# rapidsai/cugraph-gnn

Measured on AMD Instinct MI355X. Metric: sampled-edges/sec (sample+renumber+feature-gather+SAGEConv fwd), ogbn-products-like fan-out [25, 10], higher is better.
Workload: dtype int64 ids (int32 timed as a variant) + f32 features (SAGE lin_l/lin_r product: bf16x3-split MFMA, f32 accumulate); 1 GPU; ogbn-products-like RMAT: V=2449029, E=118462496 directed (CSR row_ptr i64 / col i64 replicated per GPU), feat fp32 [V,100], batch 1024/GPU, fan-out [25, 10], 2-layer SAGEConv(mean) 100-256-47 fwd, step = 8 call groups of 188 mini-batches; parallelism=dp1 (seeds sharded, no data-path collective)

## Files before the change

cugraph-gnn_amd/csrc/wg_sage_mfma.hip:

```cpp
#include "wg_sage_mfma_parts.hpp"

namespace wgamd {
namespace {
using namespace sage_mfma;

template <int TR>
__device__ __forceinline__ void consume_tile(const mfma_args& a, int64_t tile, const float* tile_lds, int cw, int lane,
                                             float* scratch)
{
  constexpr int RT = TR / 32;
  f32x16 c[RT][2];
#pragma unroll
  for (int rt = 0; rt < RT; rt++)
#pragma unroll
    for (int ct = 0; ct < 2; ct++)
#pragma unroll
      for (int i = 0; i < 16; i++) c[rt][ct][i] = 0.f;
  const int lm = lane & 31, lh = lane >> 5;
  const float* a_lane      = tile_lds + lm * a.SD + lh * 8;
  const float* b_lane = a.w_tiles + ((int64_t)(cw * 64 + lm)) * 16 + lh * 8;
  braw_t b0, b1;
  bfrag_t fb;
  araw_t<RT> raw;
  afrag_t<RT> fa;
  load_b(b0, b_lane, a.N, 0);
  for (int ks = 0; ks < a.KS; ks += 2) {
    load_a_raw<RT>(raw, a_lane, a.SD, ks);
    if (ks + 1 < a.KS) load_b(b1, b_lane, a.N, ks + 1);
    split_a<RT>(raw, fa);
    split_b(b0, fb);
    mma_frags<RT>(c, fa, fb);
    if (ks + 1 < a.KS) {
      load_a_raw<RT>(raw, a_lane, a.SD, ks + 1);
      if (ks + 2 < a.KS) load_b(b0, b_lane, a.N, ks + 2);
      split_a<RT>(raw, fa);
      split_b(b1, fb);
      mma_frags<RT>(c, fa, fb);
    }
  }
  epilogue<RT>(a, c, tile * TR, cw, lane, scratch);
}

template <int HEAD, int BODY, int VALU_PER>
__device__ __forceinline__ void mfma_valu_interleave()
{
#pragma unroll
  for (int i = 0; i < HEAD; i++) __builtin_amdgcn_sched_group_barrier(0x008, 1, 0);
#pragma unroll
  for (int i = 0; i < BODY; i++) {
    __builtin_amdgcn_sched_group_barrier(0x008, 1, 0);
    __builtin_amdgcn_sched_group_barrier(0x002, VALU_PER, 0);
  }
}

template <int RT, int AD, typename LoadA>
__device__ __forceinline__ void consume_range(const mfma_args& a, f32x16 (&c)[RT][2], bfrag_t (&b)[3], int ks0, int ks1, int cw,
                                              int lane, LoadA load_a)
{
  const int lm = lane & 31, lh = lane >> 5;
  const int64_t b_plane_dw = (int64_t)a.KS * a.N * 8;
  const uint32_t* b_lane   = reinterpret_cast<const uint32_t*>(a.w_tiles) + ((int64_t)(cw * 64 + lm)) * 8 + lh * 4;
  araw_t<RT> raw[AD];
  afrag_t<RT> fa[2];
  const int kl = ks1 - 1;
  load_a(raw[0], ks0);
  if constexpr (AD == 2) load_a(raw[1], ks0 + 1 < kl ? ks0 + 1 : kl);
  split_a<RT>(raw[0], fa[0]);
  auto step = [&](auto I, int ks) {
    constexpr int i = decltype(I)::value;
    load_a(raw[i % AD], ks + AD < kl ? ks + AD : kl);
    int kb = ks + 2;
    kb     = kb >= a.KS ? kb - a.KS : kb;
    load_b_planes(b[(i + 2) % 3], b_lane, b_plane_dw, a.N, kb);
    mma_frags<RT>(c, fa[i & 1], b[i % 3]);
    split_a<RT>(raw[(i + 1) % AD], fa[(i + 1) & 1]);
    mfma_valu_interleave<4, 6 * RT * 2 - 4, 5>();
    __builtin_amdgcn_sched_barrier(0);
  };
  int ks = ks0;
  for (; ks + 5 < ks1; ks += 6) {
    step(std::integral_constant<int, 0>{}, ks);
    step(std::integral_constant<int, 1>{}, ks + 1);
    step(std::integral_constant<int, 2>{}, ks + 2);
    step(std::integral_constant<int, 3>{}, ks + 3);
    step(std::integral_constant<int, 4>{}, ks + 4);
    step(std::integral_constant<int, 5>{}, ks + 5);
  }
  const int r = ks1 - ks;
  if (r > 0) step(std::integral_constant<int, 0>{}, ks);
  if (r > 1) step(std::integral_constant<int, 1>{}, ks + 1);
  if (r > 2) step(std::integral_constant<int, 2>{}, ks + 2);
  if (r > 3) step(std::integral_constant<int, 3>{}, ks + 3);
  if (r > 4) step(std::integral_constant<int, 4>{}, ks + 4);
  const int rot = (ks1 - ks0) % 3;
  if (rot == 1) {
    const bfrag_t t = b[0];
    b[0] = b[1], b[1] = b[2], b[2] = t;
  } else if (rot == 2) {
    const bfrag_t t = b[0];
    b[0] = b[2], b[2] = b[1], b[1] = t;
  }
}

constexpr int kPD = 2;
__host__ __device__ constexpr int b_slot(int ks) { return ks < kPD ? ks : kPD + (ks % kPD); }
__host__ __device__ constexpr int w_lds_ksteps(int FC)
{
#ifdef WG_NO_WLDS
  return 0;
#endif
  const int tiles = (2 * 64 * row_stride_dw(FC) + 16 + 4 * kScratchDw + 16) * 4;
  const int free_ = 160 * 1024 - tiles;
  const int ks    = free_ / (256 * 64);
  return ks < 0 ? 0 : (ks > 4 ? 4 : ks);
}

template <int TR, int FC>
struct static_consumer {
  static constexpr int RT = TR / 32, KSC = (2 * FC + 15) / 16, SD = row_stride_dw(FC);
  static constexpr int KL = TR == 64 ? w_lds_ksteps(FC) : 0;
  braw_t bb[2 * kPD];
  uint32_t b_lane_off;
  const float* w_lds;
  f32x16 c[RT][2];

  __device__ __forceinline__ void load_b_static(const mfma_args& a, braw_t& f, int ks) const
  {
#ifdef WG_ABL_NO_B
    return;
#endif
#ifdef WG_ABL_HALF_B
    if (ks & 1) return;
#endif
    if (ks >= KSC - KL) {
#pragma unroll
      for (int ct = 0; ct < 2; ct++)
#pragma unroll
        for (int h = 0; h < 2; h++)
          f.v[ct][h] = *reinterpret_cast<const f32x4*>(w_lds + (((ks - (KSC - KL)) * 2 + ct) * 2 + h) * 256);
      return;
    }
    const char* wb = reinterpret_cast<const char*>(a.w_tiles);
#pragma unroll
    for (int ct = 0; ct < 2; ct++) {
      const size_t at = ((size_t)ks * a.N + ct * 32) * 64 + b_lane_off;
      f.v[ct][0]      = *reinterpret_cast<const f32x4*>(wb + at);
      f.v[ct][1]      = *reinterpret_cast<const f32x4*>(wb + at + 16);
    }
  }

  __device__ __forceinline__ void prime(const mfma_args& a, int cw, int lane, float* w_lds_wave)
  {
    b_lane_off = (uint32_t)(((cw * 64 + (lane & 31)) * 16 + (lane >> 5) * 8) * 4);
    w_lds      = w_lds_wave + lane * 4;
    if constexpr (KL > 0) {
      const char* wb = reinterpret_cast<const char*>(a.w_tiles);
#pragma unroll
      for (int ks = KSC - KL; ks < KSC; ks++)
#pragma unroll
        for (int ct = 0; ct < 2; ct++)
#pragma unroll
          for (int h = 0; h < 2; h++)
            *reinterpret_cast<f32x4*>(const_cast<float*>(w_lds) + (((ks - (KSC - KL)) * 2 + ct) * 2 + h) * 256) =
              *reinterpret_cast<const f32x4*>(wb + ((size_t)ks * a.N + ct * 32) * 64 + b_lane_off + h * 16);
    }
#pragma unroll
    for (int j = 0; j < kPD; j++) load_b_static(a, bb[j], j);
  }

  __device__ __forceinline__ void multiply(const mfma_args& a, const float* tile_lds, int lane)
  {
#pragma unroll
    for (int rt = 0; rt < RT; rt++)
#pragma unroll
      for (int ct = 0; ct < 2; ct++)
#pragma unroll
        for (int i = 0; i < 16; i++) c[rt][ct][i] = 0.f;
    const float* a_lane = tile_lds + (lane & 31) * SD + (lane >> 5) * 8;
    araw_t<RT> raw;
    afrag_t<RT> fa[2];
    load_a_raw<RT>(raw, a_lane, SD, 0);
    split_a<RT>(raw, fa[0]);
#pragma unroll
    for (int ks = 0; ks < KSC; ks++) {
      if (ks + 1 < KSC) load_a_raw<RT>(raw, a_lane, SD, ks + 1);
      bfrag_t fb;
      split_b(bb[b_slot(ks)], fb);
      mma_frags<RT>(c, fa[ks & 1], fb);
      const int nk = ks + kPD;
      if (nk < KSC) load_b_static(a, bb[b_slot(nk)], nk);
      else load_b_static(a, bb[nk - KSC], nk - KSC);
      if (ks + 1 < KSC) split_a<RT>(raw, fa[(ks + 1) & 1]);
      __builtin_amdgcn_sched_barrier(0);
    }
  }
  __device__ __forceinline__ void store(const mfma_args& a, int64_t tile, int cw, int lane, float* scratch)
  {
    epilogue<RT>(a, c, tile * TR, cw, lane, scratch);
  }
};

template <typename IdT, int LG, int TR, int CW, bool OFF32, int FC, bool HALF = false>
__global__ void __launch_bounds__((CW + kProducerWaves) * 64)
sage_layer_mfma_kernel(mfma_args a)
{
  static_assert(!HALF || FC == 0, "the half-tile mode runs the runtime-shape consumer");
  extern __shared__ __attribute__((aligned(16))) float lds[];
  const int tile_dw = TR * a.SD;
  for (int i = threadIdx.x; i < 2 * tile_dw + 16; i += blockDim.x) lds[i] = 0.f;
  __syncthreads();
  const int lane = threadIdx.x & 63;
  int wave = threadIdx.x >> 6;
  if (a.debug & 64) {
    uint32_t* keys = reinterpret_cast<uint32_t*>(lds + 2 * tile_dw + 16 + CW * kScratchDw);
    const int simd = (int)__builtin_amdgcn_s_getreg((1 << 11) | (4 << 6) | 4);
    if (lane == 0) keys[wave] = (uint32_t)(((simd & 1) * 2 + (simd >> 1)) * 16 + wave);
    __syncthreads();
    const uint32_t mine_key = keys[wave];
    int rank = 0;
#pragma unroll
    for (int w = 0; w < CW + kProducerWaves; w++) rank += keys[w] < mine_key ? 1 : 0;
    wave = __builtin_amdgcn_readfirstlane(rank);
    __syncthreads();
  }
  const int64_t n_tiles = (a.n_rows + TR - 1) / TR;
  const int64_t mine    = blockIdx.x < n_tiles ? (n_tiles - blockIdx.x + gridDim.x - 1) / gridDim.x : 0;
  auto tile_of          = [&](int64_t n) { return (int64_t)blockIdx.x + n * gridDim.x; };
  auto stamp            = [&](int64_t n, int which) {
    if (a.stamps && blockIdx.x == 0 && lane == 0 && n < 64) a.stamps[(n * 8 + wave) * 2 + which] = __builtin_readcyclecounter();
  };

  if constexpr (HALF) {
    const int KSh = a.KS / 2;
    if (wave >= CW) {
      using P     = producer<IdT, LG, 32, OFF32, true>;
      using off_t = typename P::off_t;
      constexpr int IT = P::IT, kNb = P::kNb, kDepth = P::kDepth;
      static_assert(TR == 64, "two 32-row sub-tiles per tile");
      P p(a, wave - CW, lane);
      bounds_t<IT> b_next;
      ids_t<IT> i_next;
      meta_t<IT, off_t> cur;
      f32x4 buf[kDepth][kNb + 1];
      auto sub_of = [&](int64_t j) { return 2 * tile_of(j >> 1) + (j & 1); };
      p.load_bounds(sub_of(0), b_next);
      p.load_ids(sub_of(0), b_next, i_next);
      p.finish(i_next, cur);
#pragma unroll
      for (int it = 0; it < kDepth - 1; it++) p.issue(cur, it, buf[it]);
      constexpr int kHalf = IT / 2;
      for (int64_t n = 0; n <= mine; n++) {
        if (n < mine && !(a.debug & 2)) {
          float* tile_lds = lds + (n & 1) * tile_dw;
#pragma unroll
          for (int sub = 0; sub < 2; sub++) {
            const int64_t j = 2 * n + sub;
            float* rows_lds = tile_lds + sub * 32 * a.SD;
            p.load_bounds(sub_of(j + 1), b_next);
#pragma unroll
            for (int it = 0; it < IT; it++) {
              if (it == kHalf) p.load_ids(sub_of(j + 1), b_next, i_next);
              if (it + kDepth - 1 < IT) p.issue(cur, it + kDepth - 1, buf[(it + kDepth - 1) % kDepth]);
              p.reduce_store(cur, it, buf[it % kDepth], rows_lds);
            }
            p.second_window(cur, rows_lds);
            p.long_rows(sub_of(j), cur, rows_lds);
            p.finish(i_next, cur);
            if (j + 1 < 2 * mine) {
#pragma unroll
              for (int it = 0; it < kDepth - 1; it++) p.issue(cur, it, buf[it]);
            }
          }
        }
        lds_barrier();
      }
    } else {
      constexpr int RT = TR / 32;
      float* scratch = lds + 2 * tile_dw + 16 + wave * kScratchDw;
      f32x16 c[RT][2];
      bfrag_t b[3];
      {
        const uint32_t* b_lane =
          reinterpret_cast<const uint32_t*>(a.w_tiles) + ((int64_t)(wave * 64 + (lane & 31))) * 8 + (lane >> 5) * 4;
        load_b_planes(b[0], b_lane, (int64_t)a.KS * a.N * 8, a.N, 0);
        load_b_planes(b[1], b_lane, (int64_t)a.KS * a.N * 8, a.N, 1);
      }
      const IdT* src_ids = static_cast<const IdT*>(a.src_ids);
      for (int64_t n = 0; n <= mine; n++) {
        if (n >= 1 && !(a.debug & 1)) {
          const int64_t row0 = tile_of(n - 1) * TR;
          const float* self_ptr[RT];
#pragma unroll
          for (int rt = 0; rt < RT; rt++) {
            const int64_t row  = row0 + rt * 32 + (lane & 31);
            const int64_t srow = a.self_rows[row < a.n_rows ? row : a.n_rows - 1];
            self_ptr[rt]       = reinterpret_cast<const float*>(reinterpret_cast<const char*>(a.x) + table_row<IdT>(src_ids, srow) * a.row_scale) +
                           (lane >> 5) * 8;
          }
#pragma unroll
          for (int rt = 0; rt < RT; rt++)
#pragma unroll
            for (int ct = 0; ct < 2; ct++)
#pragma unroll
              for (int i = 0; i < 16; i++) c[rt][ct][i] = 0.f;
          store_agg<TR, CW>(a, lds + ((n - 1) & 1) * tile_dw, row0, wave, lane);
          const float* a_lane = lds + ((n - 1) & 1) * tile_dw + (lane & 31) * a.SD + (lane >> 5) * 8;
          consume_range<RT, 1>(a, c, b, 0, KSh, wave, lane, [&](araw_t<RT>& f, int ks) { load_a_raw<RT>(f, a_lane, a.SD, ks); });
          consume_range<RT, 2>(a, c, b, KSh, a.KS, wave, lane, [&](araw_t<RT>& f, int ks) {
#pragma unroll
            for (int rt = 0; rt < RT; rt++) {
              const float* p = self_ptr[rt] + (ks - KSh) * 16;
              f.v[rt][0]     = *reinterpret_cast<const f32x4*>(p);
              f.v[rt][1]     = *reinterpret_cast<const f32x4*>(p + 4);
            }
          });
          epilogue<RT>(a, c, row0, wave, lane, scratch);
        }
        lds_barrier();
      }
    }
  } else if (wave >= CW) {
    if (a.debug & 16) __builtin_amdgcn_s_setprio(3);
    using P     = producer<IdT, LG, TR, OFF32>;
    using off_t = typename P::off_t;
    constexpr int IT = P::IT, kNb = P::kNb, kDepth = P::kDepth;
    P p(a, wave - CW, lane);
    bounds_t<IT> b_next;
    ids_t<IT> i_next;
    meta_t<IT, off_t> cur;
    f32x4 buf[kDepth][kNb + 1];
    {
      p.load_bounds(tile_of(0), b_next);
      p.load_ids(tile_of(0), b_next, i_next);
      p.finish(i_next, cur);
    }
#pragma unroll
    for (int it = 0; it < kDepth - 1; it++) p.issue(cur, it, buf[it]);
    constexpr int kHalf = IT / 2;
    for (int64_t n = 0; n <= mine; n++) {
      stamp(n, 0);
      if (n < mine && !(a.debug & 2)) {
        float* tile_lds = lds + (n & 1) * tile_dw;
        p.load_bounds(tile_of(n + 1), b_next);
#pragma unroll
        for (int it = 0; it < IT; it++) {
          if (it == kHalf) p.load_ids(tile_of(n + 1), b_next, i_next);
          if (it + kDepth - 1 < IT) p.issue(cur, it + kDepth - 1, buf[(it + kDepth - 1) % kDepth]);
          p.reduce_store(cur, it, buf[it % kDepth], tile_lds);
        }
        p.second_window(cur, tile_lds);
        p.long_rows(tile_of(n), cur, tile_lds);
        p.finish(i_next, cur);
        if (n + 1 < mine) {
#pragma unroll
          for (int it = 0; it < kDepth - 1; it++) p.issue(cur, it, buf[it]);
        }
      }
      stamp(n, 1);
      lds_barrier();
    }
  } else {
    if (a.debug & 32) __builtin_amdgcn_s_setprio(3);
    float* scratch = lds + 2 * tile_dw + 16 + wave * kScratchDw;
    if constexpr (FC > 0) {
      static_consumer<TR, FC> cons;
      cons.prime(a, wave, lane, lds + 2 * tile_dw + 16 + CW * kScratchDw + 16 + wave * (decltype(cons)::KL * 16 * 64));
      const bool late = (wave & 1) && !(a.debug & 128);
      int64_t pending = -1;
      for (int64_t n = 0; n <= mine; n++) {
        stamp(n, 0);
        if (n >= 1 && !(a.debug & 1)) {
          const float* tile_lds = lds + ((n - 1) & 1) * tile_dw;
          store_agg<TR, CW>(a, tile_lds, tile_of(n - 1) * TR, wave, lane);
          if (late) {
            if (pending >= 0) cons.store(a, pending, wave, lane, scratch);
            cons.multiply(a, tile_lds, lane);
            pending = tile_of(n - 1);
          } else {
            cons.multiply(a, tile_lds, lane);
            cons.store(a, tile_of(n - 1), wave, lane, scratch);
          }
        }
        stamp(n, 1);
        lds_barrier();
      }
      if (late && pending >= 0) cons.store(a, pending, wave, lane, scratch);
    } else {
      for (int64_t n = 0; n <= mine; n++) {
        if (n >= 1 && !(a.debug & 1)) {
          store_agg<TR, CW>(a, lds + ((n - 1) & 1) * tile_dw, tile_of(n - 1) * TR, wave, lane);
          consume_tile<TR>(a, tile_of(n - 1), lds + ((n - 1) & 1) * tile_dw, wave, lane, scratch);
        }
        lds_barrier();
      }
    }
  }
}

__global__ void split_weight_kernel(const float* __restrict__ w_t, int64_t ldw, int K, int N, int KS, uint32_t* __restrict__ planes)
{
  const int64_t total = (int64_t)KS * N * 8;
  for (int64_t i = blockIdx.x * (int64_t)blockDim.x + threadIdx.x; i < total; i += (int64_t)gridDim.x * blockDim.x) {
    const int kk2 = (int)(i & 7);
    const int n   = (int)((i >> 3) % N);
    const int ks  = (int)((i >> 3) / N);
    const int k0  = ks * 16 + kk2 * 2;
    const float v0 = k0 < K ? w_t[(int64_t)k0 * ldw + n] : 0.f;
    const float v1 = k0 + 1 < K ? w_t[(int64_t)(k0 + 1) * ldw + n] : 0.f;
    uint32_t h0, m0, l0, h1, m1, l1;
    split3(v0, h0, m0, l0);
    split3(v1, h1, m1, l1);
    planes[i]             = pack_hi16(h0, h1);
    planes[total + i]     = pack_hi16(m0, m1);
    planes[2 * total + i] = pack_hi16(l0, l1);
  }
}

__global__ void tile_weight_kernel(const float* __restrict__ w_t, int64_t ldw, int K, int N, int KS, float* __restrict__ tiles)
{
  const int64_t total = (int64_t)KS * N * 16;
  for (int64_t i = blockIdx.x * (int64_t)blockDim.x + threadIdx.x; i < total; i += (int64_t)gridDim.x * blockDim.x) {
    const int kk = (int)(i & 15);
    const int n  = (int)((i >> 4) % N);
    const int ks = (int)((i >> 4) / N);
    const int k  = ks * 16 + kk;
    tiles[i]     = k < K ? w_t[(int64_t)k * ldw + n] : 0.f;
  }
}

__global__ void layer_weight_kernel(const float* __restrict__ w_l, int64_t ldl, const float* __restrict__ w_r, int64_t ldr,
                                    const float* __restrict__ bias, int F, int N, int Np, int KS, int half,
                                    void* __restrict__ planes_, float* __restrict__ bias_out)
{
  auto w_at = [&](int k, int n) -> float {
    if (n >= N || k >= 2 * F) return 0.f;
    return k < F ? w_l[(int64_t)n * ldl + k] : w_r[(int64_t)n * ldr + (k - F)];
  };
  const int64_t tid = blockIdx.x * (int64_t)blockDim.x + threadIdx.x, stride = (int64_t)gridDim.x * blockDim.x;
  if (bias_out)
    for (int64_t n = tid; n < Np; n += stride) bias_out[n] = (bias && n < N) ? bias[n] : 0.f;
  if (half) {
    uint32_t* planes    = static_cast<uint32_t*>(planes_);
    const int64_t total = (int64_t)KS * Np * 8;
    for (int64_t i = tid; i < total; i += stride) {
      const int kk2 = (int)(i & 7), n = (int)((i >> 3) % Np), ks = (int)((i >> 3) / Np);
      const int k0  = ks * 16 + kk2 * 2;
      uint32_t h0, m0, l0, h1, m1, l1;
      split3(w_at(k0, n), h0, m0, l0);
      split3(w_at(k0 + 1, n), h1, m1, l1);
      planes[i]             = pack_hi16(h0, h1);
      planes[total + i]     = pack_hi16(m0, m1);
      planes[2 * total + i] = pack_hi16(l0, l1);
    }
  } else {
    float* tiles        = static_cast<float*>(planes_);
    const int64_t total = (int64_t)KS * Np * 16;
    for (int64_t i = tid; i < total; i += stride) {
      const int kk = (int)(i & 15), n = (int)((i >> 4) % Np), ks = (int)((i >> 4) / Np);
      tiles[i]     = w_at(ks * 16 + kk, n);
    }
  }
}

constexpr size_t kLdsBudget = 160 * 1024;
__host__ inline size_t lds_bytes(int F, int TR) { return (size_t)(2 * TR * row_stride_dw(F) + 16 + 4 * kScratchDw + 16) * 4; }
__host__ inline size_t lds_bytes_half(int F) { return (size_t)(2 * 64 * row_stride_half_dw(F) + 16 + 4 * kScratchDw + 16) * 4; }
__host__ inline bool use_half_tiles(int F)
{
  return F % 16 == 0 && lds_bytes(F, 64) > kLdsBudget && lds_bytes_half(F) <= kLdsBudget;
}

template <typename IdT, int LG, int CW>
void launch_half(mfma_args a, hipStream_t st)
{
  const int cus         = stream_cu_count(st);
  a.SD                  = row_stride_half_dw(a.F);
  const int64_t n_tiles = (a.n_rows + 63) / 64;
  const size_t lds      = lds_bytes_half(a.F);
  const int grid        = (int)std::max<int64_t>(1, std::min<int64_t>(n_tiles, (int64_t)cus));
  auto go               = [&](auto kern) {
    WG_HIP_CHECK(hipFuncSetAttribute(reinterpret_cast<const void*>(kern), hipFuncAttributeMaxDynamicSharedMemorySize, (int)lds));
    kern<<<grid, (CW + kProducerWaves) * 64, lds, st>>>(a);
    WG_HIP_CHECK(hipGetLastError());
  };
  if (a.x_bytes != 0) go(sage_layer_mfma_kernel<IdT, LG, 64, CW, true, 0, true>);
  else go(sage_layer_mfma_kernel<IdT, LG, 64, CW, false, 0, true>);
}

template <typename IdT, int LG, int TR, int CW, int FC = 0>
void launch(const mfma_args& a, hipStream_t st)
{
  const int cus         = stream_cu_count(st);
  const int64_t n_tiles = (a.n_rows + TR - 1) / TR;
  const size_t lds      = lds_bytes(a.F, TR) + (FC > 0 && TR == 64 ? (size_t)w_lds_ksteps(FC) * CW * 64 * 64 : 0);
  const int grid = (int)std::max<int64_t>(1, std::min<int64_t>(n_tiles, (int64_t)cus));
  auto go        = [&](auto kern) {
    if (lds > 64 * 1024)
      WG_HIP_CHECK(hipFuncSetAttribute(reinterpret_cast<const void*>(kern), hipFuncAttributeMaxDynamicSharedMemorySize, (int)lds));
    kern<<<grid, (CW + kProducerWaves) * 64, lds, st>>>(a);
    WG_HIP_CHECK(hipGetLastError());
  };
  if (a.x_bytes != 0) go(sage_layer_mfma_kernel<IdT, LG, TR, CW, true, FC>);
  else go(sage_layer_mfma_kernel<IdT, LG, TR, CW, false, FC>);
}

template <typename IdT, int LG, int TR>
void launch_cw(const mfma_args& a, hipStream_t st)
{
  switch (a.N / 64) {
    case 1: launch<IdT, LG, TR, 1>(a, st); break;
    case 2: launch<IdT, LG, TR, 2>(a, st); break;
    default:
      if constexpr (LG == 32 && TR == 64) {
        if (a.F == 100) return launch<IdT, LG, TR, 4, 100>(a, st);
        if (a.F == 128) return launch<IdT, LG, TR, 4, 128>(a, st);
      }
      launch<IdT, LG, TR, 4>(a, st);
      break;
  }
}

template <typename IdT, int LG>
void launch_tr(const mfma_args& a, hipStream_t st)
{
  if constexpr (LG <= 32) {
    launch_cw<IdT, LG, 64>(a, st);
  } else {
    if (use_half_tiles(a.F) && !a.full_tiles) {
      switch (a.N / 64) {
        case 1: launch_half<IdT, LG, 1>(a, st); break;
        case 2: launch_half<IdT, LG, 2>(a, st); break;
        default: launch_half<IdT, LG, 4>(a, st); break;
      }
    } else launch_cw<IdT, LG, 32>(a, st);
  }
}

template <typename IdT>
void launch_groups(const mfma_args& a, hipStream_t st)
{
  const int units = a.F / 4;
  if (units <= 8) launch_tr<IdT, 8>(a, st);
  else if (units <= 16) launch_tr<IdT, 16>(a, st);
  else if (units <= 32) launch_tr<IdT, 32>(a, st);
  else launch_tr<IdT, 64>(a, st);
}

}
}

#ifndef WG_MFMA_TUNE_HARNESS
extern "C" size_t wgamd_sage_weight_planes_bytes(int K, int N) { return (size_t)3 * ((K + 15) / 16) * (size_t)N * 32; }

extern "C" int wgamd_sage_layer_bf16x3_supported(int F, int N)
{
  return F > 0 && F % 4 == 0 && F <= 256 && (N == 64 || N == 128 || N == 256) && wgamd::lds_bytes(F, 32) <= wgamd::kLdsBudget;
}

extern "C" wholememory_error_code_t wgamd_sage_split_weight_bf16x3(const float* w_t, int64_t ldw, int K, int N, void* planes,
                                                                   void* stream)
{
  using namespace wgamd;
  return guarded("wgamd_sage_split_weight_bf16x3", [&] {
    WG_REQUIRE_INPUT(w_t && planes && K > 0 && N > 0 && ldw >= N, "bad weight");
    const int KS        = (K + 15) / 16;
    const int64_t total = (int64_t)KS * N * 16;
    const int grid      = (int)std::min<int64_t>((total + 255) / 256, 2048);
    if (K % 2 == 0 && use_half_tiles(K / 2))
      split_weight_kernel<<<grid, 256, 0, static_cast<hipStream_t>(stream)>>>(w_t, ldw, K, N, KS, static_cast<uint32_t*>(planes));
    else
      tile_weight_kernel<<<grid, 256, 0, static_cast<hipStream_t>(stream)>>>(w_t, ldw, K, N, KS, static_cast<float*>(planes));
    WG_HIP_CHECK(hipGetLastError());
  });
}

extern "C" int wgamd_sage_layer_uses_half_tiles(int F) { return wgamd::use_half_tiles(F) ? 1 : 0; }

extern "C" wholememory_error_code_t wgamd_sage_layer_weight_planes(const float* w_l, int64_t ldl, const float* w_r, int64_t ldr,
                                                                  const float* bias, int F, int N, int Np, void* planes,
                                                                  float* bias_out, int full_tiles, void* stream)
{
  using namespace wgamd;
  return guarded("wgamd_sage_layer_weight_planes", [&] {
    WG_REQUIRE_INPUT(w_l && w_r && planes && F > 0 && N > 0 && Np >= N && ldl >= F && ldr >= F, "bad weights");
    const int K = 2 * F, KS = (K + 15) / 16;
    const int half      = (use_half_tiles(F) && !full_tiles) ? 1 : 0;
    const int64_t total = (int64_t)KS * Np * 16;
    const int grid      = (int)std::min<int64_t>((total + 255) / 256, 2048);
    layer_weight_kernel<<<grid, 256, 0, static_cast<hipStream_t>(stream)>>>(w_l, ldl, w_r, ldr, bias, F, N, Np, KS, half, planes, bias_out);
    WG_HIP_CHECK(hipGetLastError());
  });
}

extern "C" wholememory_error_code_t wgamd_sage_layer_fused_bf16x3(const int* row_ptr, const int* col, int64_t n_rows,
                                                                  const float* x, int64_t ldx, int64_t x_rows, int F,
                                                                  const void* src_ids, wholememory_dtype_t src_ids_dtype,
                                                                  const int64_t* self_rows, int mean, const void* w_planes,
                                                                  int N, const float* bias, int relu, float* out, int64_t ldo,
                                                                  void* stream)
{
  return wgamd_sage_layer_fused_bf16x3_train(row_ptr, col, n_rows, x, ldx, x_rows, F, src_ids, src_ids_dtype, self_rows, mean,
                                             w_planes, N, bias, relu, out, ldo, nullptr, 0, stream);
}

extern "C" wholememory_error_code_t wgamd_sage_layer_fused_bf16x3_train(const int* row_ptr, const int* col, int64_t n_rows,
                                                                        const float* x, int64_t ldx, int64_t x_rows, int F,
                                                                        const void* src_ids, wholememory_dtype_t src_ids_dtype,
                                                                        const int64_t* self_rows, int mean, const void* w_planes,
                                                                        int N, const float* bias, int relu, float* out,
                                                                        int64_t ldo, float* agg_out, int64_t ld_agg, void* stream)
{
  using namespace wgamd;
  return guarded("wgamd_sage_layer_fused_bf16x3", [&] {
    WG_REQUIRE_INPUT(n_rows >= 0 && F > 0 && N > 0, "bad sizes");
    if (n_rows == 0) return;
    WG_REQUIRE_INPUT(row_ptr && col && x && self_rows && w_planes && out, "null pointer");
    if (!wgamd_sage_layer_bf16x3_supported(F, N) || ldx % 4 != 0 || (reinterpret_cast<uintptr_t>(x) & 15) != 0)
      throw logic_error(fmt("unsupported shape: F=%d (multiple of 4, <= 256), N=%d (64, 128 or 256), 16-B aligned rows", F, N));
    WG_REQUIRE_INPUT(ldo >= N, "leading dimension smaller than N");
    if (ldo % 4 != 0 || (reinterpret_cast<uintptr_t>(out) & 15) != 0) throw logic_error("output rows must be 16-B aligned");
    if (agg_out != nullptr && (ld_agg < F || ld_agg % 4 != 0 || (reinterpret_cast<uintptr_t>(agg_out) & 15) != 0))
      throw logic_error("agg_out rows must hold F floats and be 16-B aligned");
    const uint64_t xb = x_rows > 0 ? (uint64_t)x_rows * (uint64_t)ldx * 4u : 0;
    mfma_args a{row_ptr, col, n_rows, x, ldx, (uint32_t)(xb > 0 && xb < (1ull << 31) ? xb : 0), F, src_ids, self_rows, mean,
                static_cast<const float*>(w_planes), N, (2 * F + 15) / 16, bias, relu & 1, out, ldo, row_stride_dw(F), 0, nullptr,
                ldx * 4, agg_out, ld_agg, (relu & WGAMD_SAGE_FULL_TILES) != 0};
    const bool byte_offsets = src_ids != nullptr && src_ids_dtype == WGAMD_IDS_BYTE_OFFSETS;
    if (byte_offsets) {
      a.row_scale = 1;
      a.x_bytes   = 0;
    }
    auto st = static_cast<hipStream_t>(stream);
    if (src_ids == nullptr) launch_groups<void>(a, st);
    else if (src_ids_dtype == WHOLEMEMORY_DT_INT) launch_groups<int32_t>(a, st);
    else if (src_ids_dtype == WHOLEMEMORY_DT_INT64 || byte_offsets) launch_groups<int64_t>(a, st);
    else throw invalid_input("src_ids must be INT, INT64 or WGAMD_IDS_BYTE_OFFSETS");
  });
}
#endif
```

cugraph-gnn_amd/csrc/wg_sage_mfma_parts.hpp:

```cpp
#pragma once
#include <algorithm>
#include <cstdlib>
#include <type_traits>

#include "wg_common.hpp"
#include "wgamd_ext.h"

namespace wgamd {
namespace sage_mfma {

using f32x4  = __attribute__((ext_vector_type(4))) float;
using f32x16 = __attribute__((ext_vector_type(16))) float;
using u32x4  = __attribute__((ext_vector_type(4))) uint32_t;
using bf16x8 = __attribute__((ext_vector_type(8))) __bf16;

#ifndef WG_MFMA_PRODUCTS
#define WG_MFMA_PRODUCTS 6
#endif
#ifndef WG_MFMA_DEPTH
#define WG_MFMA_DEPTH 2
#endif
constexpr int kProducerWaves = 4;
constexpr int kRingDepth     = WG_MFMA_DEPTH;

template <typename IdT>
__device__ __forceinline__ int64_t table_row(const IdT* ids, int64_t local)
{
  if constexpr (std::is_same<IdT, void>::value) return local;
  else return (int64_t)ids[local];
}

struct mfma_args {
  const int* row_ptr;
  const int* col;
  int64_t n_rows;
  const float* x;
  int64_t ldx;
  uint32_t x_bytes;
  int F;
  const void* src_ids;
  const int64_t* self_rows;
  int mean;
  const float* w_tiles;
  int N;
  int KS;
  const float* bias;
  int relu;
  float* out;
  int64_t ldo;
  int SD;
  int debug;
  unsigned long long* stamps;
  int64_t row_scale;
  float* agg_out;
  int64_t ld_agg;
  int full_tiles;
};

__device__ __forceinline__ void split3(float a, uint32_t& h, uint32_t& m, uint32_t& l)
{
  h              = __float_as_uint(a) & 0xffff0000u;
  const float r1 = a - __uint_as_float(h);
  m              = __float_as_uint(r1) & 0xffff0000u;
  const float r2 = r1 - __uint_as_float(m);
  l              = __float_as_uint(r2);
}
__device__ __forceinline__ uint32_t pack_hi16(uint32_t a, uint32_t b) { return __builtin_amdgcn_perm(b, a, 0x07060302u); }

__device__ __forceinline__ void lds_barrier() { asm volatile("s_waitcnt lgkmcnt(0)\n\ts_barrier" ::: "memory"); }

__host__ __device__ constexpr int row_stride_dw(int F)
{
  int sd = (2 * F + 3) / 4 * 4;
  return (sd / 4) % 2 == 0 ? sd + 4 : sd;
}

__host__ __device__ constexpr int row_stride_half_dw(int F)
{
  int sd = (F + 3) / 4 * 4;
  return (sd / 4) % 2 == 0 ? sd + 4 : sd;
}

template <int IT>
struct bounds_t {
  int s[IT], e[IT];
};
template <int IT>
struct ids_t {
  int deg[IT];
  int lcol[IT];
  int lself[IT];
};
template <int IT, typename off_t>
struct meta_t {
  int d[IT];
  off_t src[IT];
  off_t self[IT];
};

template <typename IdT, int LG, int TR, bool OFF32, bool HALF = false>
struct producer {
  using off_t                         = typename std::conditional<OFF32, uint32_t, int64_t>::type;
  static constexpr int kGroupsPerWave = 64 / LG;
  static constexpr int kGroups        = kGroupsPerWave * kProducerWaves;
  static constexpr int IT             = TR / kGroups;
  static constexpr int kNb            = LG < 10 ? LG : 10;
  static constexpr int kDepth         = IT < kRingDepth ? IT : kRingDepth;
  static_assert(TR % kGroups == 0, "lane groups must tile the rows evenly");

  const mfma_args& a;
  const int sub, gbase, group, f0, f0c;
  const bool live;
  __amdgpu_buffer_rsrc_t rsrc;

  __device__ producer(const mfma_args& a_, int pw, int lane)
    : a(a_),
      sub(lane & (LG - 1)),
      gbase(lane & ~(LG - 1)),
      group(pw * kGroupsPerWave + lane / LG),
      f0((lane & (LG - 1)) * 4),
      f0c(((lane & (LG - 1)) * 4 < a_.F) ? (lane & (LG - 1)) * 4 : a_.F - 4),
      live((lane & (LG - 1)) * 4 < a_.F),
      rsrc(__builtin_amdgcn_make_buffer_rsrc(const_cast<float*>(a_.x), 0, (int)a_.x_bytes, 0x00020000))
  {
  }

  __device__ __forceinline__ int64_t row_of(int64_t tile, int it) const { return tile * TR + group + it * kGroups; }

  __device__ __forceinline__ void load_bounds(int64_t tile, bounds_t<IT>& b) const
  {
#pragma unroll
    for (int it = 0; it < IT; it++) {
      const int64_t row  = row_of(tile, it);
      const int64_t rowc = row < a.n_rows ? row : a.n_rows - 1;
      b.s[it]            = a.row_ptr[rowc];
      b.e[it]            = a.row_ptr[rowc + 1];
    }
  }
  __device__ __forceinline__ void load_ids(int64_t tile, const bounds_t<IT>& b, ids_t<IT>& v) const
  {
#pragma unroll
    for (int it = 0; it < IT; it++) {
      const int64_t row = row_of(tile, it);
      v.deg[it]         = row < a.n_rows ? b.e[it] - b.s[it] : -1;
      const int* pc     = (sub < b.e[it] - b.s[it]) ? a.col + b.s[it] + sub : a.row_ptr;
      v.lcol[it]        = *pc;
      v.lself[it]       = (int)a.self_rows[row < a.n_rows ? row : a.n_rows - 1];
    }
  }
  __device__ __forceinline__ void finish(const ids_t<IT>& v, meta_t<IT, off_t>& m) const
  {
    const IdT* src_ids = static_cast<const IdT*>(a.src_ids);
#pragma unroll
    for (int it = 0; it < IT; it++) {
      m.d[it]    = v.deg[it];
      m.src[it]  = (off_t)(table_row<IdT>(src_ids, (int64_t)v.lcol[it]) * a.row_scale);
      m.self[it] = (off_t)(table_row<IdT>(src_ids, (int64_t)v.lself[it]) * a.row_scale);
    }
  }
  __device__ __forceinline__ void issue(const meta_t<IT, off_t>& m, int it, f32x4* v) const
  {
#ifndef WG_ISSUE_READLANE64
#define WG_ISSUE_READLANE64 1
#endif
#ifndef WG_ISSUE_DPP
#define WG_ISSUE_DPP 1
#endif
#ifndef WG_ISSUE_BPERMUTE
    if constexpr (LG == 32 && WG_ISSUE_DPP) {
      issue_dpp(m, it, v);
      return;
    }
    if constexpr (LG == 32 || (LG == 64 && WG_ISSUE_READLANE64)) {
      issue_all<0>(m, it, v);
      return;
    }
#endif
    if constexpr (OFF32) {
#pragma unroll
      for (int k = 0; k < kNb; k++) {
        const uint32_t off = (uint32_t)__shfl((int)m.src[it], gbase | (k & (LG - 1)), 64);
        v[k] = __builtin_bit_cast(f32x4, __builtin_amdgcn_raw_buffer_load_b128(rsrc, k < m.d[it] ? off + f0c * 4 : a.x_bytes, 0, 0));
      }
      if constexpr (!HALF)
        v[kNb] = __builtin_bit_cast(
          f32x4, __builtin_amdgcn_raw_buffer_load_b128(rsrc, m.d[it] >= 0 ? (uint32_t)m.self[it] + f0c * 4 : a.x_bytes, 0, 0));
    } else {
      const char* xb = reinterpret_cast<const char*>(a.x);
#pragma unroll
      for (int k = 0; k < kNb; k++) {
        const int src_lane = gbase | (k & (LG - 1));
        const int lo       = __shfl((int)(m.src[it] & 0xffffffff), src_lane, 64);
        const int hi       = __shfl((int)((int64_t)m.src[it] >> 32), src_lane, 64);
        int64_t off        = ((int64_t)hi << 32) | (uint32_t)lo;
        off                = k < m.d[it] ? off : (int64_t)0;
        v[k]               = *reinterpret_cast<const f32x4*>(xb + off + f0c * 4);
      }
      if constexpr (!HALF)
        v[kNb] = *reinterpret_cast<const f32x4*>(xb + (m.d[it] >= 0 ? (int64_t)m.self[it] : (int64_t)0) + f0c * 4);
    }
  }
  template <int k>
  __device__ __forceinline__ void issue_dpp_one(const meta_t<IT, off_t>& m, int it, f32x4* v, int dlo, int dhi) const
  {
    if constexpr (k < kNb) {
      const int lo = __builtin_amdgcn_update_dpp(0, dlo, 0x150 + k, 0xf, 0xf, false);
      if constexpr (OFF32) {
        v[k] = __builtin_bit_cast(
          f32x4, __builtin_amdgcn_raw_buffer_load_b128(rsrc, k < m.d[it] ? (uint32_t)lo + f0c * 4 : a.x_bytes, 0, 0));
      } else {
        const int hi      = __builtin_amdgcn_update_dpp(0, dhi, 0x150 + k, 0xf, 0xf, false);
        const int64_t off = ((int64_t)hi << 32) | (uint32_t)lo;
        v[k]              = *reinterpret_cast<const f32x4*>(reinterpret_cast<const char*>(a.x) + off + f0c * 4);
      }
      issue_dpp_one<k + 1>(m, it, v, dlo, dhi);
    }
  }
  __device__ __forceinline__ void issue_dpp(const meta_t<IT, off_t>& m, int it, f32x4* v) const
  {
    static_assert(kNb <= 16, "the first window sits in the even row of the group");
    const int slo = (int)((uint64_t)m.src[it] & 0xffffffffu);
    const int dlo = __builtin_amdgcn_permlane16_swap(slo, slo, false, false)[0];
    int dhi       = 0;
    if constexpr (!OFF32) {
      const int shi = (int)((uint64_t)m.src[it] >> 32);
      dhi           = __builtin_amdgcn_permlane16_swap(shi, shi, false, false)[0];
    }
    issue_dpp_one<0>(m, it, v, dlo, dhi);
    if constexpr (!HALF) issue_one<kNb>(m, it, v);
  }
  template <int k>
  __device__ __forceinline__ int group_lane(int v) const
  {
    if constexpr (LG == 32) {
      const int lo = __builtin_amdgcn_readlane(v, k), hi = __builtin_amdgcn_readlane(v, 32 + k);
      return gbase ? hi : lo;
    } else if constexpr (LG == 64) {
      return __builtin_amdgcn_readlane(v, k);
    } else {
      return __shfl(v, gbase | (k & (LG - 1)), 64);
    }
  }
  template <int k>
  __device__ __forceinline__ void issue_all(const meta_t<IT, off_t>& m, int it, f32x4* v) const
  {
    if constexpr (k < kNb + (HALF ? 0 : 1)) {
      issue_one<k>(m, it, v);
      issue_all<k + 1>(m, it, v);
    }
  }
  template <int k>
  __device__ __forceinline__ void issue_one(const meta_t<IT, off_t>& m, int it, f32x4* v) const
  {
    static_assert(!HALF || k < kNb, "no self slot in half-tile mode");
    if constexpr (OFF32) {
      if constexpr (k < kNb) {
        const uint32_t off = (uint32_t)group_lane<k>((int)m.src[it]);
        v[k] = __builtin_bit_cast(f32x4, __builtin_amdgcn_raw_buffer_load_b128(rsrc, k < m.d[it] ? off + f0c * 4 : a.x_bytes, 0, 0));
      } else {
        v[kNb] = __builtin_bit_cast(
          f32x4, __builtin_amdgcn_raw_buffer_load_b128(rsrc, m.d[it] >= 0 ? (uint32_t)m.self[it] + f0c * 4 : a.x_bytes, 0, 0));
      }
    } else {
      const char* xb = reinterpret_cast<const char*>(a.x);
      if constexpr (k < kNb) {
        const int lo = group_lane<k>((int)(m.src[it] & 0xffffffff));
        const int hi = group_lane<k>((int)((int64_t)m.src[it] >> 32));
        int64_t off  = ((int64_t)hi << 32) | (uint32_t)lo;
        off          = k < m.d[it] ? off : (int64_t)0;
        v[k]         = *reinterpret_cast<const f32x4*>(xb + off + f0c * 4);
      } else {
        v[kNb] = *reinterpret_cast<const f32x4*>(xb + (m.d[it] >= 0 ? (int64_t)m.self[it] : (int64_t)0) + f0c * 4);
      }
    }
  }
  __device__ __forceinline__ void reduce_store(const meta_t<IT, off_t>& m, int it, const f32x4* v, float* tile_lds) const
  {
    const int deg = m.d[it];
    f32x4 acc     = {0.f, 0.f, 0.f, 0.f};
#pragma unroll
    for (int k = 0; k < kNb; k++) {
      if constexpr (OFF32) acc += v[k];
      else acc += k < deg ? v[k] : f32x4{0.f, 0.f, 0.f, 0.f};
    }
    if (a.mean && deg > 0 && deg <= kNb) acc *= __frcp_rn((float)deg);
    if (live) {
      float* prow = tile_lds + (group + it * kGroups) * a.SD;
      *reinterpret_cast<f32x4*>(prow + f0) = acc;
      if constexpr (!HALF) {
        f32x4 self = v[kNb];
        if constexpr (!OFF32) self = deg >= 0 ? self : f32x4{0.f, 0.f, 0.f, 0.f};
        *reinterpret_cast<f32x4*>(prow + a.F + f0) = self;
      }
    }
  }
  static constexpr int kW2 = LG >= 32 ? 16 : (LG > kNb ? LG - kNb : 0);
  __device__ __forceinline__ void second_window(const meta_t<IT, off_t>& m, float* tile_lds) const
  {
    if constexpr (kW2 > 0) {
#pragma unroll
      for (int it = 0; it < IT; it++) {
        const int deg = m.d[it];
        if (__ballot(deg > kNb) == 0ull) continue;
        const bool mine = live && deg > kNb;
        f32x4 v[kW2];
#pragma unroll
        for (int k = 0; k < kW2; k++) {
          const int kk = kNb + k;
          if constexpr (OFF32) {
            const uint32_t off = (uint32_t)__shfl((int)m.src[it], gbase | kk, 64);
            v[k] = __builtin_bit_cast(f32x4, __builtin_amdgcn_raw_buffer_load_b128(rsrc, kk < deg ? off + f0c * 4 : a.x_bytes, 0, 0));
          } else {
            const int lo = __shfl((int)(m.src[it] & 0xffffffff), gbase | kk, 64);
            const int hi = __shfl((int)((int64_t)m.src[it] >> 32), gbase | kk, 64);
            int64_t off  = ((int64_t)hi << 32) | (uint32_t)lo;
            off          = kk < deg ? off : (int64_t)0;
            v[k]         = *reinterpret_cast<const f32x4*>(reinterpret_cast<const char*>(a.x) + off + f0c * 4);
          }
        }
        float* prow = tile_lds + (group + it * kGroups) * a.SD + f0;
        f32x4 acc   = {0.f, 0.f, 0.f, 0.f};
        if (mine) acc = *reinterpret_cast<const f32x4*>(prow);
#pragma unroll
        for (int k = 0; k < kW2; k++) {
          if constexpr (OFF32) acc += v[k];
          else acc += kNb + k < deg ? v[k] : f32x4{0.f, 0.f, 0.f, 0.f};
        }
        if (mine) {
          if (a.mean && deg <= kNb + kW2) acc *= __frcp_rn((float)deg);
          *reinterpret_cast<f32x4*>(prow) = acc;
        }
      }
    }
  }
  static constexpr int kLongUnroll = 8;
  __device__ __forceinline__ void long_rows(int64_t tile, const meta_t<IT, off_t>& m, float* tile_lds) const
  {
    long_rows_from<kNb + kW2, kLongUnroll>(tile, m, tile_lds);
  }
  template <int kStart, int kUnroll>
  __device__ __forceinline__ void long_rows_from(int64_t tile, const meta_t<IT, off_t>& m, float* tile_lds) const
  {
    const IdT* src_ids = static_cast<const IdT*>(a.src_ids);
#pragma unroll
    for (int it = 0; it < IT; it++) {
      const int deg = m.d[it];
      if (__ballot(deg > kStart) == 0ull) continue;
      const bool mine    = live && deg > kStart;
      const int64_t row  = row_of(tile, it);
      const int64_t rowc = row < a.n_rows ? row : a.n_rows - 1;
      const int s        = a.row_ptr[rowc];
      float* prow        = tile_lds + (group + it * kGroups) * a.SD + f0;
      f32x4 acc          = {0.f, 0.f, 0.f, 0.f};
      if (mine) acc = *reinterpret_cast<const f32x4*>(prow);
      int maxdeg = deg > kStart ? deg : 0;
#pragma unroll
      for (int dd = 32; dd >= LG; dd >>= 1) maxdeg = max(maxdeg, __shfl_xor(maxdeg, dd, 64));
      for (int c0 = kStart; c0 < maxdeg; c0 += LG) {
        const int64_t my_src = (deg > kStart && c0 + sub < deg) ? table_row<IdT>(src_ids, (int64_t)a.col[s + c0 + sub]) : 0;
// ... 187 lines not shown
```

Before: 5.292 billion sampled-edges/s.

## Replace static tile striding with atomic ticket-based dynamic tile scheduling

The persistent SAGE layer kernel stops assigning tiles to blocks by fixed stride and instead draws the next tile from a global atomic counter, passing it through a small LDS ring from the producer wave to the consumers. This targets load imbalance from skewed node degrees, where some blocks finish their fixed share early and idle. It adds an atomic per tile, extra LDS reads and readfirstlane broadcasts, a host-side per-stream ticket slot allocator, and a counter reset at kernel end that relies on every block finishing.

Measured after the change: 5.352 billion sampled-edges/s (median of 6 runs). 1.01x the previous value.

```diff
diff --git a/cugraph-gnn_amd/csrc/wg_sage_mfma.hip b/cugraph-gnn_amd/csrc/wg_sage_mfma.hip
--- a/cugraph-gnn_amd/csrc/wg_sage_mfma.hip
+++ b/cugraph-gnn_amd/csrc/wg_sage_mfma.hip
@@ -207,7 +207,11 @@
   static_assert(!HALF || FC == 0, "the half-tile mode runs the runtime-shape consumer");
   extern __shared__ __attribute__((aligned(16))) float lds[];
   const int tile_dw = TR * a.SD;
+  uint32_t* ring = reinterpret_cast<uint32_t*>(lds + 2 * tile_dw + 16 + CW * kScratchDw) + 8;
+  uint32_t first_ticket = kNoTile;
+  if (threadIdx.x == 0 && (int64_t)blockIdx.x < (a.n_rows + TR - 1) / TR) first_ticket = (uint32_t)gridDim.x + atomicAdd(a.tickets, 1u);
   for (int i = threadIdx.x; i < 2 * tile_dw + 16; i += blockDim.x) lds[i] = 0.f;
+  if (threadIdx.x == 0) ring[0] = blockIdx.x, ring[1] = first_ticket;
   __syncthreads();
   const int lane = threadIdx.x & 63;
   int wave = threadIdx.x >> 6;
@@ -223,9 +227,19 @@
     wave = __builtin_amdgcn_readfirstlane(rank);
     __syncthreads();
   }
-  const int64_t n_tiles = (a.n_rows + TR - 1) / TR;
-  const int64_t mine    = blockIdx.x < n_tiles ? (n_tiles - blockIdx.x + gridDim.x - 1) / gridDim.x : 0;
-  auto tile_of          = [&](int64_t n) { return (int64_t)blockIdx.x + n * gridDim.x; };
+  const uint32_t n_tiles = (uint32_t)((a.n_rows + TR - 1) / TR);
+  const bool drawer      = wave == CW && lane == 0;
+  auto draw              = [&](uint32_t known) {
+    return known < n_tiles ? (uint32_t)gridDim.x + atomicAdd(a.tickets, 1u) : kNoTile;
+  };
+  auto ring_at = [&](int r) { return (uint32_t)__builtin_amdgcn_readfirstlane((int)ring[r]); };
+  uint32_t t_prev = kNoTile, t_cur = ring_at(0);
+  int r_next = 1;
+  auto advance = [&](uint32_t t_next) {
+    t_prev = t_cur, t_cur = t_next;
+    r_next = r_next == 2 ? 0 : r_next + 1;
+  };
+  auto r_draw = [&] { return r_next == 2 ? 0 : r_next + 1; };
   auto stamp            = [&](int64_t n, int which) {
     if (a.stamps && blockIdx.x == 0 && lane == 0 && n < 64) a.stamps[(n * 8 + wave) * 2 + which] = __builtin_readcyclecounter();
   };
@@ -242,37 +256,42 @@
       ids_t<IT> i_next;
       meta_t<IT, off_t> cur;
       f32x4 buf[kDepth][kNb + 1];
-      auto sub_of = [&](int64_t j) { return 2 * tile_of(j >> 1) + (j & 1); };
-      p.load_bounds(sub_of(0), b_next);
-      p.load_ids(sub_of(0), b_next, i_next);
+      p.load_bounds(2 * (int64_t)t_cur, b_next);
+      p.load_ids(2 * (int64_t)t_cur, b_next, i_next);
       p.finish(i_next, cur);
 #pragma unroll
       for (int it = 0; it < kDepth - 1; it++) p.issue(cur, it, buf[it]);
       constexpr int kHalf = IT / 2;
-      for (int64_t n = 0; n <= mine; n++) {
-        if (n < mine && !(a.debug & 2)) {
+      for (int n = 0;; n++) {
+        const uint32_t t_next = ring_at(r_next);
+        uint32_t drawn       = kNoTile;
+        if (drawer && t_cur < n_tiles) drawn = draw(t_next);
+        if (t_cur < n_tiles && !(a.debug & 2)) {
           float* tile_lds = lds + (n & 1) * tile_dw;
 #pragma unroll
           for (int sub = 0; sub < 2; sub++) {
-            const int64_t j = 2 * n + sub;
+            const int64_t s_cur = 2 * (int64_t)t_cur + sub, s_next = sub == 0 ? s_cur + 1 : 2 * (int64_t)t_next;
             float* rows_lds = tile_lds + sub * 32 * a.SD;
-            p.load_bounds(sub_of(j + 1), b_next);
+            p.load_bounds(s_next, b_next);
 #pragma unroll
             for (int it = 0; it < IT; it++) {
-              if (it == kHalf) p.load_ids(sub_of(j + 1), b_next, i_next);
+              if (it == kHalf) p.load_ids(s_next, b_next, i_next);
               if (it + kDepth - 1 < IT) p.issue(cur, it + kDepth - 1, buf[(it + kDepth - 1) % kDepth]);
               p.reduce_store(cur, it, buf[it % kDepth], rows_lds);
             }
             p.second_window(cur, rows_lds);
-            p.long_rows(sub_of(j), cur, rows_lds);
+            p.long_rows(s_cur, cur, rows_lds);
+            if (sub == 1 && drawer) ring[r_draw()] = drawn;
             p.finish(i_next, cur);
-            if (j + 1 < 2 * mine) {
+            if (sub == 0 || t_next < n_tiles) {
 #pragma unroll
               for (int it = 0; it < kDepth - 1; it++) p.issue(cur, it, buf[it]);
             }
           }
-        }
+        } else if (drawer) ring[r_draw()] = drawn;
         lds_barrier();
+        if (t_cur >= n_tiles) break;
+        advance(t_next);
       }
     } else {
       constexpr int RT = TR / 32;
@@ -286,9 +305,10 @@
         load_b_planes(b[1], b_lane, (int64_t)a.KS * a.N * 8, a.N, 1);
       }
       const IdT* src_ids = static_cast<const IdT*>(a.src_ids);
-      for (int64_t n = 0; n <= mine; n++) {
+      for (int n = 0;; n++) {
+        const uint32_t t_next = ring_at(r_next);
         if (n >= 1 && !(a.debug & 1)) {
-          const int64_t row0 = tile_of(n - 1) * TR;
+          const int64_t row0 = (int64_t)t_prev * TR;
           const float* self_ptr[RT];
 #pragma unroll
           for (int rt = 0; rt < RT; rt++) {
@@ -317,6 +337,8 @@
           epilogue<RT>(a, c, row0, wave, lane, scratch);
         }
         lds_barrier();
+        if (t_cur >= n_tiles) break;
+        advance(t_next);
       }
     }
   } else if (wave >= CW) {
@@ -330,34 +352,40 @@
     meta_t<IT, off_t> cur;
     f32x4 buf[kDepth][kNb + 1];
     {
-      p.load_bounds(tile_of(0), b_next);
-      p.load_ids(tile_of(0), b_next, i_next);
+      p.load_bounds(t_cur, b_next);
+      p.load_ids(t_cur, b_next, i_next);
       p.finish(i_next, cur);
     }
 #pragma unroll
     for (int it = 0; it < kDepth - 1; it++) p.issue(cur, it, buf[it]);
     constexpr int kHalf = IT / 2;
-    for (int64_t n = 0; n <= mine; n++) {
+    for (int n = 0;; n++) {
       stamp(n, 0);
-      if (n < mine && !(a.debug & 2)) {
+      const uint32_t t_next = ring_at(r_next);
+      uint32_t drawn       = kNoTile;
+      if (drawer && t_cur < n_tiles) drawn = draw(t_next);
+      if (t_cur < n_tiles && !(a.debug & 2)) {
         float* tile_lds = lds + (n & 1) * tile_dw;
-        p.load_bounds(tile_of(n + 1), b_next);
+        p.load_bounds(t_next, b_next);
 #pragma unroll
         for (int it = 0; it < IT; it++) {
-          if (it == kHalf) p.load_ids(tile_of(n + 1), b_next, i_next);
+          if (it == kHalf) p.load_ids(t_next, b_next, i_next);
           if (it + kDepth - 1 < IT) p.issue(cur, it + kDepth - 1, buf[(it + kDepth - 1) % kDepth]);
           p.reduce_store(cur, it, buf[it % kDepth], tile_lds);
         }
         p.second_window(cur, tile_lds);
-        p.long_rows(tile_of(n), cur, tile_lds);
+        p.long_rows(t_cur, cur, tile_lds);
+        if (drawer) ring[r_draw()] = drawn;
         p.finish(i_next, cur);
-        if (n + 1 < mine) {
+        if (t_next < n_tiles) {
 #pragma unroll
           for (int it = 0; it < kDepth - 1; it++) p.issue(cur, it, buf[it]);
         }
-      }
+      } else if (drawer) ring[r_draw()] = drawn;
       stamp(n, 1);
       lds_barrier();
+      if (t_cur >= n_tiles) break;
+      advance(t_next);
     }
   } else {
     if (a.debug & 32) __builtin_amdgcn_s_setprio(3);
@@ -367,33 +395,43 @@
       cons.prime(a, wave, lane, lds + 2 * tile_dw + 16 + CW * kScratchDw + 16 + wave * (decltype(cons)::KL * 16 * 64));
       const bool late = (wave & 1) && !(a.debug & 128);
       int64_t pending = -1;
-      for (int64_t n = 0; n <= mine; n++) {
+      for (int n = 0;; n++) {
         stamp(n, 0);
+        const uint32_t t_next = ring_at(r_next);
         if (n >= 1 && !(a.debug & 1)) {
           const float* tile_lds = lds + ((n - 1) & 1) * tile_dw;
-          store_agg<TR, CW>(a, tile_lds, tile_of(n - 1) * TR, wave, lane);
+          store_agg<TR, CW>(a, tile_lds, (int64_t)t_prev * TR, wave, lane);
           if (late) {
             if (pending >= 0) cons.store(a, pending, wave, lane, scratch);
             cons.multiply(a, tile_lds, lane);
-            pending = tile_of(n - 1);
+            pending = t_prev;
           } else {
             cons.multiply(a, tile_lds, lane);
-            cons.store(a, tile_of(n - 1), wave, lane, scratch);
+            cons.store(a, t_prev, wave, lane, scratch);
           }
         }
         stamp(n, 1);
         lds_barrier();
+        if (t_cur >= n_tiles) break;
+        advance(t_next);
       }
       if (late && pending >= 0) cons.store(a, pending, wave, lane, scratch);
     } else {
-      for (int64_t n = 0; n <= mine; n++) {
+      for (int n = 0;; n++) {
+        const uint32_t t_next = ring_at(r_next);
         if (n >= 1 && !(a.debug & 1)) {
-          store_agg<TR, CW>(a, lds + ((n - 1) & 1) * tile_dw, tile_of(n - 1) * TR, wave, lane);
-          consume_tile<TR>(a, tile_of(n - 1), lds + ((n - 1) & 1) * tile_dw, wave, lane, scratch);
+          store_agg<TR, CW>(a, lds + ((n - 1) & 1) * tile_dw, (int64_t)t_prev * TR, wave, lane);
+          consume_tile<TR>(a, t_prev, lds + ((n - 1) & 1) * tile_dw, wave, lane, scratch);
         }
         lds_barrier();
+        if (t_cur >= n_tiles) break;
+        advance(t_next);
       }
     }
+  }
+  if (threadIdx.x == 0 && atomicAdd(a.tickets + 1, 1u) == gridDim.x - 1) {
+    atomicExch(a.tickets, 0u);
+    atomicExch(a.tickets + 1, 0u);
   }
 }
 
@@ -462,6 +500,47 @@
   }
 }
 
+constexpr int kSlotsPerBlock = 512;
+__host__ inline uint32_t* ticket_slot(hipStream_t st)
+{
+  struct key_t {
+    int dev;
+    hipStream_t st;
+    unsigned long long capture;
+    bool operator<(const key_t& o) const { return std::tie(dev, st, capture) < std::tie(o.dev, o.st, o.capture); }
+  };
+  struct block_t {
+    uint32_t* base;
+    int used;
+  };
+  static std::mutex m;
+  static std::map<key_t, uint32_t*> slot_of;
+  static std::map<int, block_t> block_of;
+  key_t key{0, st, 0};
+  WG_HIP_CHECK(hipGetDevice(&key.dev));
+  hipStreamCaptureStatus status = hipStreamCaptureStatusNone;
+  if (st != nullptr) WG_HIP_CHECK(hipStreamGetCaptureInfo(st, &status, &key.capture));
+  if (status != hipStreamCaptureStatusActive) key.capture = 0;
+  std::lock_guard<std::mutex> g(m);
+  auto it = slot_of.find(key);
+  if (it != slot_of.end()) return it->second;
+  block_t& b = block_of[key.dev];
+  if (b.base == nullptr || b.used == kSlotsPerBlock) {
+    hipStreamCaptureMode mode = hipStreamCaptureModeRelaxed;
+    WG_HIP_CHECK(hipThreadExchangeStreamCaptureMode(&mode));
+    void* p             = nullptr;
+    const hipError_t e1 = hipMalloc(&p, kSlotsPerBlock * 2 * sizeof(uint32_t));
+    const hipError_t e2 = e1 == hipSuccess ? hipMemset(p, 0, kSlotsPerBlock * 2 * sizeof(uint32_t)) : e1;
+    WG_HIP_CHECK(hipThreadExchangeStreamCaptureMode(&mode));
+    WG_HIP_CHECK(e1);
+    WG_HIP_CHECK(e2);
+    b = block_t{static_cast<uint32_t*>(p), 0};
+  }
+  uint32_t* slot = b.base + 2 * b.used++;
+  slot_of.emplace(key, slot);
+  return slot;
+}
+
 constexpr size_t kLdsBudget = 160 * 1024;
 __host__ inline size_t lds_bytes(int F, int TR) { return (size_t)(2 * TR * row_stride_dw(F) + 16 + 4 * kScratchDw + 16) * 4; }
 __host__ inline size_t lds_bytes_half(int F) { return (size_t)(2 * 64 * row_stride_half_dw(F) + 16 + 4 * kScratchDw + 16) * 4; }
@@ -474,6 +553,7 @@
 void launch_half(mfma_args a, hipStream_t st)
 {
   const int cus         = stream_cu_count(st);
+  a.tickets             = ticket_slot(st);
   a.SD                  = row_stride_half_dw(a.F);
   const int64_t n_tiles = (a.n_rows + 63) / 64;
   const size_t lds      = lds_bytes_half(a.F);
@@ -488,9 +568,10 @@
 }
 
 template <typename IdT, int LG, int TR, int CW, int FC = 0>
-void launch(const mfma_args& a, hipStream_t st)
+void launch(mfma_args a, hipStream_t st)
 {
   const int cus         = stream_cu_count(st);
+  a.tickets             = ticket_slot(st);
   const int64_t n_tiles = (a.n_rows + TR - 1) / TR;
   const size_t lds      = lds_bytes(a.F, TR) + (FC > 0 && TR == 64 ? (size_t)w_lds_ksteps(FC) * CW * 64 * 64 : 0);
   const int grid = (int)std::max<int64_t>(1, std::min<int64_t>(n_tiles, (int64_t)cus));
@@ -618,6 +699,7 @@
     if (!wgamd_sage_layer_bf16x3_supported(F, N) || ldx % 4 != 0 || (reinterpret_cast<uintptr_t>(x) & 15) != 0)
       throw logic_error(fmt("unsupported shape: F=%d (multiple of 4, <= 256), N=%d (64, 128 or 256), 16-B aligned rows", F, N));
     WG_REQUIRE_INPUT(ldo >= N, "leading dimension smaller than N");
+    WG_REQUIRE_INPUT(n_rows < ((int64_t)1 << 36), "too many rows for 32-bit tile numbers");
     if (ldo % 4 != 0 || (reinterpret_cast<uintptr_t>(out) & 15) != 0) throw logic_error("output rows must be 16-B aligned");
     if (agg_out != nullptr && (ld_agg < F || ld_agg % 4 != 0 || (reinterpret_cast<uintptr_t>(agg_out) & 15) != 0))
       throw logic_error("agg_out rows must hold F floats and be 16-B aligned");
diff --git a/cugraph-gnn_amd/csrc/wg_sage_mfma_parts.hpp b/cugraph-gnn_amd/csrc/wg_sage_mfma_parts.hpp
--- a/cugraph-gnn_amd/csrc/wg_sage_mfma_parts.hpp
+++ b/cugraph-gnn_amd/csrc/wg_sage_mfma_parts.hpp
@@ -1,6 +1,9 @@
 #pragma once
 #include <algorithm>
 #include <cstdlib>
+#include <map>
+#include <mutex>
+#include <tuple>
 #include <type_traits>
 
 #include "wg_common.hpp"
@@ -21,6 +24,7 @@
 #define WG_MFMA_DEPTH 2
 #endif
 constexpr int kProducerWaves = 4;
+constexpr uint32_t kNoTile   = 0xffffffffu;
 constexpr int kRingDepth     = WG_MFMA_DEPTH;
 
 template <typename IdT>
@@ -55,6 +59,7 @@
   float* agg_out;
   int64_t ld_agg;
   int full_tiles;
+  uint32_t* tickets;
 };
 
 __device__ __forceinline__ void split3(float a, uint32_t& h, uint32_t& m, uint32_t& l)
```
